# dylanpeifer/deepgroebner

Measured on NVIDIA B200. Metric: env_steps_per_sec, higher is better.
Workload: dtype u64 packed monomials + u32 GF(32003) coefficients (integer)

## Files before the change

### deepgroebner_b200/csrc/bb_device.cuh

```cuda
#pragma once
#include <cuda_runtime.h>
#include <stdint.h>

#include "../../include/bbenv.h"
#include "bb_layout.cuh"

#define BB_FULL 0xffffffffu
#ifndef BB_ADD_BASIS_INLINE
#define BB_ADD_BASIS_INLINE __noinline__
#endif
#define BB_GOLD 0x9E3779B97F4A7C15ULL
#define BB_GOLD2 0xD1B54A32D192ED03ULL

struct __align__(16) BBEnvState {
  int nG, nP, nT, status;
  int steps, adds, zero, nonzero;
  int rerolls, episode, truncated;
  unsigned sel_rng;
  unsigned long long trace_hash;
  unsigned long long rng;
  double disc_return, discount;
  unsigned long long pad2[2];
};

// ... 589 lines not shown
    if (two && i1 < m) { r1 = rlm[i1]; x1 = ridx[i1]; }
    pos = __popc(__ballot_sync(BB_FULL, i0 < m && r0 >= fk));
    if (two) pos += __popc(__ballot_sync(BB_FULL, i1 < m && r1 >= fk));
    __syncwarp();
    if (i0 < m && i0 >= pos) { rlm[i0 + 1] = r0; ridx[i0 + 1] = x0; }
    if (two && i1 < m && i1 >= pos) { rlm[i1 + 1] = r1; ridx[i1 + 1] = x1; }
    __syncwarp();
  } else if (H.sort_reducers) {
    int cnt = 0;
#pragma unroll 1
    for (int b0 = 0; b0 < m; b0 += 32) {
      const int r = b0 + lane;
      cnt += __popc(__ballot_sync(BB_FULL, r < m && rlm[r] >= fk));
    }
    pos = cnt;
#pragma unroll 1
    for (int hi = m; hi > pos; hi -= 32) {
      const int lo = hi - 32 > pos ? hi - 32 : pos;
      const int idx = lo + lane;
      const bool v = idx < hi;
      uint64_t k = 0; uint32_t ix = 0;
      if (v) { k = rlm[idx]; ix = ridx[idx]; }
      __syncwarp();
      if (v) { rlm[idx + 1] = k; ridx[idx + 1] = ix; }
      __syncwarp();
    }
  }
  if (lane == 0) {
    rlm[pos] = fk; ridx[pos] = (uint32_t)m;
    lm[m] = fk;
    GHeadMem* g = reinterpret_cast<GHeadMem*>(base + H.o_ghead) + m;
    if constexpr (TWO) {
      tk[0] = fk; tc[0] = c0;
      if (len > 1) { tk[1] = k1; tc[1] = c1; }
      else { k1 = 0ull; c1 = 0u; }
    }
    const uint32_t inv = bb_global(H.invtab)[TWO ? c0 : tc[0]];
    if constexpr (!TWO) {
      k1 = len > 1 ? tk[1] : 0ull;
      c1 = len > 1 ? tc[1] : 0u;
    }
    reinterpret_cast<uint4*>(g)[0] = make_uint4((uint32_t)fk, (uint32_t)(fk >> 32), (uint32_t)k1, (uint32_t)(k1 >> 32));
    reinterpret_cast<uint4*>(g)[1] = make_uint4(inv | (c1 << 16), (uint32_t)sug, (uint32_t)off, (uint32_t)len);
  }
  __syncwarp();
  return ((long long)emitted << 32) | (long long)nP;
}
template <int NV>
__device__ BB_ADD_BASIS_INLINE long long warp_add_basis(const BBParams& P, unsigned char* base, int m, int nP, int off, int len,
                                                        int sug) {
  return add_basis_body<NV, false>(P, base, m, nP, off, len, sug, 0ull, 0ull, 0u, 0u);
}
template <int NV>
__device__ BB_ADD_BASIS_INLINE long long warp_add_basis(const BBParams& P, unsigned char* base, int m, int nP, int off, int len,
                                                        int sug, uint64_t fk, uint64_t k1, uint32_t c0, uint32_t c1) {
  return add_basis_body<NV, true>(P, base, m, nP, off, len, sug, fk, k1, c0, c1);
}

__device__ __forceinline__ void warp_take_pair(const BBParams& P, Env& e, int row, uint32_t& pr, uint64_t& gam) {
  const int lane = bb_lane();
  uint32_t* pairs = ENV_PTR(uint32_t, e, P, o_pairs);
  uint64_t* plcm = ENV_PTR(uint64_t, e, P, o_plcm);
  pr = pairs[row];
  gam = plcm[row];
  __syncwarp();
#pragma unroll 1
  for (int b0 = row; b0 < e.nP - 1; b0 += 32) {
    const int idx = b0 + lane;
    const bool v = idx < e.nP - 1;
    uint32_t x = 0u; uint64_t y = 0ull;
    if (v) { x = pairs[idx + 1]; y = plcm[idx + 1]; }
    __syncwarp();
    if (v) { pairs[idx] = x; plcm[idx] = y; }
  }
  e.nP--;
}

template <int NV, bool TWO = false>
__device__ __forceinline__ int warp_step(const BBParams& P, Env& e, int row, uint32_t& pair, Ctr& ct) {
  typedef KL<NV> K;
  const BBField F = P.F;
  if ((unsigned)row >= (unsigned)e.nP) { e.status = BB_STATUS_BAD_ACTION; pair = 0xffffffffu; return 0; }
  uint32_t pr; uint64_t gam;
  warp_take_pair(P, e, row, pr, gam);
  const int i = pr & 0xffffu, j = pr >> 16;
  pair = pr;
  const GHeadMem* gh = ENV_PTR(GHeadMem, e, P, o_ghead);
  const GHead hf = load_head(gh + i), hg = load_head(gh + j);
  e.guard |= gam;
  ct.tread += hf.len + hg.len;
  Dividend h;
  h.k0 = h.k1 = 0; h.c0 = h.c1 = 0; h.n = 0; h.loc = -1;
  {
    const int cg0 = (int)(uint32_t)(gam >> K::dshift);
    const int sf = (int)hf.sug + (int)(uint32_t)(hf.lm >> K::dshift) - cg0, sg = (int)hg.sug + (int)(uint32_t)(hg.lm >> K::dshift) - cg0;
    h.sug = sf > sg ? sf : sg;
  }
  const uint64_t adjf = gam - hf.lm, adjg = gam - hg.lm;
  const uint32_t cg = F.p - hg.invlc;
  if (TWO || (hf.len <= 2 && hg.len <= 2)) {
    const uint64_t ka = hf.k1 + adjf, kb = hg.k1 + adjg;
    const bool hasA = hf.len == 2, hasB = hg.len == 2;
    if (hasA) e.guard |= ka;
    if (hasB) e.guard |= kb;
    tiny_merge(F, hasA, ka, bbf_mulmod(F, hf.c1, hf.invlc), hasB, kb, bbf_mulmod(F, hg.c1, cg), h);
  } else if constexpr (!TWO) {
    const uint64_t* tk = ENV_PTR(uint64_t, e, P, o_tkey);
// ... 506 lines not shown
```

### deepgroebner_b200/csrc/bb_kernels.cuh

```cuda
#pragma once
#include "bb_device.cuh"
#include "bb_policy.cuh"
#include "bb_streams.cuh"
#if defined(BBW_CLOCK) || defined(BBW_INSTR)
#include <cstdio>
#endif
#include "bb_wide.cuh"
#include "bb_rstreams.cuh"

#ifndef BB_WARPS
#define BB_WARPS 8
#endif
#define BB_THREADS (BB_WARPS * 32)
#ifndef BB_MIN_BLOCKS
#define BB_MIN_BLOCKS 3
#endif

#ifndef BB_ROLLOUT_MIN_BLOCKS
#define BB_ROLLOUT_MIN_BLOCKS 2
#endif

struct BBRunArgs {
  int strategy, episodes, seed_base;
  int sel_seed_base;
  int sel_seed_stride;
  int ep_base;
  int ep_offset;
  int nstaged;
  const int* seeds;
  int max_steps;
  double gamma;
  int compute_gb;
  bb_poly_sink gb_sink, basis_sink;
  bb_episode_stats* out;
  int32_t* trace;
  int trace_eps, trace_cap;
  int prepare_by_warp;
  int stream_kmax;
  int stream_regs;
  int ctl_reducers;
  int* queue;
  int* order;
  uint8_t* cost_key;
  int two_term;
};
#define BB_LPT_BUCKETS 256
#define BB_LPT_HIST 4

#define BB_PREP_S 16
struct BBPre {
  BBParams S;
  int depth;
  int* count;
  int* head;
  unsigned* rng;
  int* calls;
};

struct BBEpisodeAcc {
  unsigned long long th;
  double ret, disc;
  uint32_t sel_rng, pad;
};

struct BBValueArgs {
  int strategy;
  int rollouts;
  int sel_seed_base;
// ... 1 lines not shown
  double gamma;
  double* value;
  int* queue;
  int ntasks;
};

struct BBRolloutArgs {
  BBPolicy W;
  int T;
  unsigned long long counter0;
  int32_t* actions; float* logp; float* reward; uint8_t* done; int32_t* lengths;
  int32_t* obs; int pmax;
};

enum { BB_CMD_STEP = 1, BB_CMD_RESET = 2, BB_CMD_OBSERVE = 3, BB_CMD_STOP = 4 };
struct BBMailbox {
  volatile unsigned cmd_seq;
  unsigned cmd;
  int arg;
  int rows;
  unsigned pad0[12];
  volatile unsigned done_seq;
  volatile unsigned alive;
  int length;
  unsigned done;
  double reward;
  unsigned pad1[10];
};
static_assert(sizeof(BBMailbox) == 128, "mailbox header is two 64-byte lines");

struct BBKernelTable {
  int nvars, w, dw, dshift, eshift;
  cudaError_t (*reset)(const BBParams&, const uint8_t* mask, int nwarps, cudaStream_t);
  cudaError_t (*step)(const BBParams&, const int* actions, double* reward, uint8_t* done, const int* active, int nwarps,
                      cudaStream_t);
  cudaError_t (*step_obs)(const BBParams&, const int* actions, int action0, double* reward, uint8_t* done, int32_t* obs,
                          int32_t* lengths, int pmax, int pad, int do_step, const int* active, unsigned* ready, unsigned ticket,
                          int nwarps, cudaStream_t);
  cudaError_t (*serve)(const BBParams&, BBMailbox* mb, unsigned long long idle_ns, cudaStream_t);
  cudaError_t (*prefill)(const BBParams&, const BBParams& stage, int period, cudaStream_t);
  cudaError_t (*select)(const BBParams&, int strategy, int* actions, int nwarps, cudaStream_t);
  cudaError_t (*observe)(const BBParams&, int32_t* obs, int32_t* lengths, int pmax, int nwarps, cudaStream_t);
  cudaError_t (*final_gb)(const BBParams&, int slot, int* ok_out, cudaStream_t);
  cudaError_t (*prepare)(const BBParams& stage, const BBRunArgs&, cudaStream_t);
  cudaError_t (*run)(const BBParams&, const BBParams& stage, const BBRunArgs&, int nwarps, cudaStream_t);
  cudaError_t (*run_streams)(const BBParams&, const BBParams& stage, const BBRunArgs&, int nwarps, cudaStream_t);
  int (*streams_warps_per_sm)(void);
  cudaError_t (*run_wide)(const BBParams&, const BBParams& stage, const BBRunArgs&, int nctas, cudaStream_t);
  int (*wide_ctas_per_sm)(void);
  cudaError_t (*value)(const BBParams&, const BBParams& fork, const BBValueArgs&, int nwarps, cudaStream_t);
  cudaError_t (*policy)(const BBParams&, const BBPolicy&, unsigned long long counter, int32_t* actions, float* logp,
                        float* logits, int pmax, int nwarps, cudaStream_t);
  cudaError_t (*rollout)(const BBParams&, const BBRolloutArgs&, int nwarps, cudaStream_t);
  int (*run_blocks_per_sm)(void);
};

const BBKernelTable* bb_kernel_table(int nvars);

#ifdef BB_NV

__device__ __forceinline__ void counters_flush(const BBParams& P, unsigned long long (*sh)[CT_COUNT]) {
  __syncthreads();
  if (threadIdx.x < CT_COUNT) {
    unsigned long long s = 0;
#pragma unroll
    for (int w = 0; w < BB_WARPS; w++) s += sh[w][threadIdx.x];
    if (s) atomicAdd(&P.counters[threadIdx.x], s);
  }
}
__device__ __forceinline__ unsigned long long* counters_row(unsigned long long (*sh)[CT_COUNT]) {
  unsigned long long* row = sh[threadIdx.x >> 5];
  if (bb_lane() < CT_COUNT) row[bb_lane()] = 0ull;
  __syncwarp();
  return row;
}

template <int NV>
__device__ __noinline__ void warp_next_episode(const BBParams& P, int slot, unsigned long long* row);

template <int NV>
__global__ void __launch_bounds__(BB_THREADS, BB_MIN_BLOCKS) k_reset(const __grid_constant__ BBParams P, const uint8_t* mask) {
  __shared__ unsigned long long sh[BB_WARPS][CT_COUNT];
  hot_init(P);
  unsigned long long* row = counters_row(sh);
  const int slot = (blockIdx.x * BB_THREADS + threadIdx.x) >> 5;
  if (slot < P.num_envs && (!mask || mask[slot])) warp_next_episode<NV>(P, slot, row);
  counters_flush(P, sh);
}

template <int NV>
__device__ __forceinline__ double step_and_account(const BBParams& P, int slot, Env& e, int action, Ctr& ct,
                                                   unsigned long long* row) {
  uint32_t pr;
  const int g0 = e.nG;
  const int adds = warp_step<NV>(P, e, action, pr, ct);
  if (pr == 0xffffffffu) return 0.0;
  if (bb_lane() == 0) {
    const int pi = pr & 0xffffu, pj = pr >> 16;
    BBEnvState& S = P.st[slot];
    S.trace_hash = trace_hash_step(S.trace_hash, pr, adds);
    S.steps += 1; S.adds += adds;
    if (e.nG > g0) S.nonzero += 1; else S.zero += 1;
    row[CT_STEPS] += 1; row[CT_ADDS] += (unsigned)adds;
    row[e.nG > g0 ? CT_NONZERO : CT_ZERO] += 1;
    if (e.status == BB_STATUS_DONE) row[CT_EPISODES] += 1;
  }
  if (P.max_episode_length > 0 && e.status == BB_STATUS_RUNNING) {
// ... 533 lines not shown
      int steps = 0, adds = 0;
      if (lane == 0) { acc.th = 0ull; acc.ret = 0.0; acc.disc = 1.0; acc.sel_rng = rng_seed(A.sel_seed_base + (A.ep_offset + ep) * A.sel_seed_stride); }
      __syncwarp();
      run_episode<NV, STREAMS, TWO>(P, e, A.strategy, A.max_steps, A.gamma, acc, ct, steps, adds,
                               (A.trace && ep < A.trace_eps) ? reinterpret_cast<int4*>(A.trace) + (size_t)ep * A.trace_cap : nullptr,
                               A.trace_cap, &ws);
      const int nonzero = e.nG - g_start, zero = steps - nonzero;
      env_store(P, slot, e);
      __syncwarp();
      const GHeadMem* gh = ENV_PTR(GHeadMem, e, P, o_ghead);
      const unsigned long long bh = warp_terms_hash<NV>(ENV_PTR(uint64_t, e, P, o_tkey), ENV_PTR(uint32_t, e, P, o_tcoef),
                                                        e.nT, reinterpret_cast<const int*>(&gh[0].len),
                                                        (int)(sizeof(GHeadMem) / sizeof(int)), e.nG);
      unsigned long long gbh = 0; int gp = 0, gt = 0;
      int status = e.status;
      if (A.compute_gb && status == BB_STATUS_DONE) {
        if (warp_final_gb<NV>(P, slot, row)) {
          gp = P.gcount[2 * slot]; gt = P.gcount[2 * slot + 1];
          gbh = warp_terms_hash<NV>(P.gkey + (size_t)slot * P.max_terms, P.gcoef + (size_t)slot * P.max_terms, gt,
                                    P.glen + (size_t)slot * P.max_basis, 1, gp);
        } else {
          status = BB_STATUS_OVERFLOW_SCRATCH;
        }
      }
      if (EXPORT && (A.gb_sink.lens_dev || A.basis_sink.lens_dev)) warp_export_episode<NV>(P, A, slot, ep, status);
      if (lane == 0) {
        const unsigned long long th = acc.th; const double ret = acc.ret;
        bb_episode_stats o;
        o.steps = steps; o.additions = adds; o.zero_reductions = zero; o.nonzero_reductions = nonzero;
        o.nbasis = e.nG; o.nterms = e.nT; o.status = status; o.rerolls = S.st[b].rerolls;
        o.trace_hash = th; o.basis_hash = bh; o.gb_hash = gbh; o.gb_polys = gp; o.gb_terms = gt;
        o.discounted_return = ret;
        A.out[ep] = o;
        BBEnvState& St = P.st[slot];
        St.status = status; St.steps = steps; St.adds = adds; St.zero = zero; St.nonzero = nonzero; St.trace_hash = th;
        St.disc_return = ret; St.rerolls = o.rerolls;
        row[CT_STEPS] += (unsigned)steps; row[CT_ADDS] += (unsigned)adds; row[CT_NONZERO] += (unsigned)nonzero;
        row[CT_ZERO] += (unsigned)zero; row[CT_EPISODES] += 1;
      }
      ct.spill(row);
      __syncwarp();
    }
  }
  __syncthreads();
  if (threadIdx.x < CT_COUNT) {
    unsigned long long s = 0;
#pragma unroll
    for (int w = 0; w < WARPS; w++) s += sh[w][threadIdx.x];
    if (s) atomicAdd(&P.counters[threadIdx.x], s);
  }
}

template <int NV, bool EXPORT = false, bool TWO = false>
__global__ void __launch_bounds__(BB_THREADS, BB_MIN_BLOCKS) k_run(const __grid_constant__ BBParams P,
                                                                  const __grid_constant__ BBParams S,
                                                                  const __grid_constant__ BBRunArgs A) {
  run_worker<NV, false, BB_WARPS, EXPORT, TWO>(P, S, A);
}

#ifndef BBS_WARPS
#define BBS_WARPS 4
#endif
#ifndef BBS_MIN_CTAS
#define BBS_MIN_CTAS 2
#endif
template <int NV, bool EXPORT = false>
__global__ void __launch_bounds__(BBS_WARPS * 32, BBS_MIN_CTAS) k_run_streams(const __grid_constant__ BBParams P,
                                                                             const __grid_constant__ BBParams S,
                                                                             const __grid_constant__ BBRunArgs A) {
  run_worker<NV, true, BBS_WARPS, EXPORT>(P, S, A);
}

__device__ __forceinline__ void block_copy_words(uint32_t* __restrict__ d, const uint32_t* __restrict__ s, int n) {
  d = bb_global(d); s = bb_global(s);
#pragma unroll 1
  for (int t = threadIdx.x; t < n; t += BBW_THREADS) d[t] = s[t];
}

template <int NV>
__global__ void __launch_bounds__(BBW_THREADS, BBW_MIN_CTAS) k_run_wide(const __grid_constant__ BBParams P, const __grid_constant__ BBParams S,
                                                          const __grid_constant__ BBRunArgs A) {
  extern __shared__ __align__(16) unsigned char wide_smem[];
  __shared__ unsigned long long sh[1][CT_COUNT];
  __shared__ BBEpisodeAcc acc;
  __shared__ WideShared wsh;
  __shared__ int next_b;
  WideStreams& st = *reinterpret_cast<WideStreams*>(wide_smem);
  const int tid = threadIdx.x;
  const int slot = blockIdx.x;
  hot_init(P);
  if (tid < CT_COUNT) sh[0][tid] = 0ull;
  __syncthreads();
  unsigned long long* row = sh[0];
  Ctr ct; ct.clear();
  WideState ws;
  ws.clear(); ws.cz = 0;
#ifdef BBW_INSTR
  ws.n_rounds = ws.n_trounds = ws.sum_T = ws.n_consol = ws.n_crounds = ws.n_topen = 0;
#endif
#ifdef BBW_CLOCK
  ws.cw = ws.cb = ws.cp = ws.co = ws.s_sel = ws.s_take = ws.s_red = ws.s_upd = 0; ws.tl = clock64();
#endif
  ws.regs = A.stream_regs < BBW_SLOTS ? (A.stream_regs < 2 ? 2 : A.stream_regs) : BBW_SLOTS;
  ws.cbase = A.ctl_reducers >= 32 && A.ctl_reducers < 256 ? (A.ctl_reducers & ~31) : 256;
  ws.tcap = A.stream_kmax - ws.regs < 0 ? 0 : (A.stream_kmax - ws.regs < BBW_KMAX - BBW_THREADS ? A.stream_kmax - ws.regs : BBW_KMAX - BBW_THREADS);
  int half = 0;
  for (;;) {
    if (tid == 0) { int q = atomicAdd(A.queue, 1); next_b = q < A.episodes ? A.order[q] : -1; }
    __syncthreads();
    const int b = next_b;
// ... 198 lines not shown
      }
    }
    env_store(P, slot, e);
    ct.spill(row);
  }
  counters_flush(P, sh);
}

static inline int grid_for_warps(int nwarps) { return (nwarps + BB_WARPS - 1) / BB_WARPS; }

template <int NV>
struct BBLaunch {
  static cudaError_t reset(const BBParams& P, const uint8_t* mask, int nwarps, cudaStream_t s) {
    k_reset<NV><<<grid_for_warps(nwarps), BB_THREADS, 0, s>>>(P, mask);
    return cudaGetLastError();
  }
  static cudaError_t step(const BBParams& P, const int* actions, double* reward, uint8_t* done, const int* active, int nwarps,
                          cudaStream_t s) {
    k_step<NV><<<grid_for_warps(nwarps), BB_THREADS, 0, s>>>(P, actions, reward, done, active);
    return cudaGetLastError();
  }
  static cudaError_t step_obs(const BBParams& P, const int* actions, int action0, double* reward, uint8_t* done, int32_t* obs,
                              int32_t* lengths, int pmax, int pad, int do_step, const int* active, unsigned* ready,
                              unsigned ticket, int nwarps, cudaStream_t s) {
    k_step_obs<NV><<<grid_for_warps(nwarps), BB_THREADS, 0, s>>>(P, actions, action0, reward, done, obs, lengths, pmax, pad, do_step,
                                                                active, ready, ticket);
    return cudaGetLastError();
  }
  static cudaError_t serve(const BBParams& P, BBMailbox* mb, unsigned long long idle_ns, cudaStream_t s) {
    k_serve<NV><<<1, 32, 0, s>>>(P, mb, idle_ns);
    return cudaGetLastError();
  }
  static cudaError_t prefill(const BBParams& P, const BBParams& S, int period, cudaStream_t s) {
    k_prefill<NV><<<(P.num_envs + BB_PREP_THREADS - 1) / BB_PREP_THREADS, BB_PREP_THREADS, 0, s>>>(P, S, period);
    return cudaGetLastError();
  }
  static cudaError_t select(const BBParams& P, int strategy, int* actions, int nwarps, cudaStream_t s) {
    k_select<NV><<<grid_for_warps(nwarps), BB_THREADS, 0, s>>>(P, strategy, actions);
    return cudaGetLastError();
  }
  static cudaError_t observe(const BBParams& P, int32_t* obs, int32_t* lengths, int pmax, int nwarps, cudaStream_t s) {
    k_observe<NV><<<grid_for_warps(nwarps), BB_THREADS, 0, s>>>(P, obs, lengths, pmax);
    return cudaGetLastError();
  }
  static cudaError_t final_gb(const BBParams& P, int slot, int* ok_out, cudaStream_t s) {
    k_final_gb<NV><<<1, 32, 0, s>>>(P, slot, ok_out);
    return cudaGetLastError();
  }
  static void same_carveout() {
    static bool done = false;
    if (done) return;
    done = true;
    const int pct = 7;
    cudaFuncSetAttribute(k_run<NV>, cudaFuncAttributePreferredSharedMemoryCarveout, pct);
    cudaFuncSetAttribute(k_run<NV, true>, cudaFuncAttributePreferredSharedMemoryCarveout, pct);
    cudaFuncSetAttribute(k_run<NV, false, true>, cudaFuncAttributePreferredSharedMemoryCarveout, pct);
    cudaFuncSetAttribute(k_run<NV, true, true>, cudaFuncAttributePreferredSharedMemoryCarveout, pct);
    cudaFuncSetAttribute(k_prepare<NV>, cudaFuncAttributePreferredSharedMemoryCarveout, pct);
    cudaFuncSetAttribute(k_prepare_lanes<NV>, cudaFuncAttributePreferredSharedMemoryCarveout, pct);
    cudaFuncSetAttribute(k_order<NV>, cudaFuncAttributePreferredSharedMemoryCarveout, pct);
  }
  static cudaError_t prepare(const BBParams& S, const BBRunArgs& A, cudaStream_t s) {
    same_carveout();
    if (S.dist.enabled && S.dist.kind == 0 && S.dist.s <= BB_PREP_S && !A.prepare_by_warp)
      k_prepare_lanes<NV><<<(A.episodes + BB_PREP_THREADS - 1) / BB_PREP_THREADS, BB_PREP_THREADS, 0, s>>>(S, A);
    else
      k_prepare<NV><<<grid_for_warps(A.episodes), BB_THREADS, 0, s>>>(S, A);
    k_order<NV><<<std::min(64, (A.episodes + 1023) / 1024), BB_LPT_BUCKETS, 0, s>>>(A);
    return cudaGetLastError();
  }
  static cudaError_t run(const BBParams& P, const BBParams& S, const BBRunArgs& A, int nwarps, cudaStream_t s) {
    same_carveout();
    const bool ex = A.gb_sink.lens_dev || A.basis_sink.lens_dev;
    if (A.two_term) {
      if (ex) k_run<NV, true, true><<<grid_for_warps(nwarps), BB_THREADS, 0, s>>>(P, S, A);
      else k_run<NV, false, true><<<grid_for_warps(nwarps), BB_THREADS, 0, s>>>(P, S, A);
    } else {
      if (ex) k_run<NV, true><<<grid_for_warps(nwarps), BB_THREADS, 0, s>>>(P, S, A);
      else k_run<NV><<<grid_for_warps(nwarps), BB_THREADS, 0, s>>>(P, S, A);
    }
    return cudaGetLastError();
  }
  static size_t streams_smem() { return 0; }
  static int streams_warps_per_sm() {
    const size_t sm = streams_smem();
    if (cudaFuncSetAttribute(k_run_streams<NV>, cudaFuncAttributeMaxDynamicSharedMemorySize, (int)sm) != cudaSuccess) return 0;
    int blocks = 0;
    if (cudaOccupancyMaxActiveBlocksPerMultiprocessor(&blocks, k_run_streams<NV>, BBS_WARPS * 32, sm) != cudaSuccess) return 0;
    return blocks * BBS_WARPS;
  }
  static cudaError_t run_streams(const BBParams& P, const BBParams& S, const BBRunArgs& A, int nwarps, cudaStream_t s) {
    const size_t sm = streams_smem();
    const bool ex = A.gb_sink.lens_dev || A.basis_sink.lens_dev;
    cudaError_t e = cudaFuncSetAttribute(ex ? k_run_streams<NV, true> : k_run_streams<NV>,
                                         cudaFuncAttributeMaxDynamicSharedMemorySize, (int)sm);
    if (e != cudaSuccess) return e;
    if (ex) k_run_streams<NV, true><<<(nwarps + BBS_WARPS - 1) / BBS_WARPS, BBS_WARPS * 32, sm, s>>>(P, S, A);
    else k_run_streams<NV><<<(nwarps + BBS_WARPS - 1) / BBS_WARPS, BBS_WARPS * 32, sm, s>>>(P, S, A);
    return cudaGetLastError();
  }
  static int wide_ctas_per_sm() {
    const size_t sm = sizeof(WideStreams);
    if (cudaFuncSetAttribute(k_run_wide<NV>, cudaFuncAttributeMaxDynamicSharedMemorySize, (int)sm) != cudaSuccess) return 0;
    int blocks = 0;
    if (cudaOccupancyMaxActiveBlocksPerMultiprocessor(&blocks, k_run_wide<NV>, BBW_THREADS, sm) != cudaSuccess) return 0;
    return blocks;
  }
  static cudaError_t run_wide(const BBParams& P, const BBParams& S, const BBRunArgs& A, int nctas, cudaStream_t s) {
    const size_t sm = sizeof(WideStreams);
    cudaError_t e = cudaFuncSetAttribute(k_run_wide<NV>, cudaFuncAttributeMaxDynamicSharedMemorySize, (int)sm);
    if (e != cudaSuccess) return e;
    k_run_wide<NV><<<nctas, BBW_THREADS, sm, s>>>(P, S, A);
    return cudaGetLastError();
  }
  static cudaError_t value(const BBParams& P, const BBParams& F, const BBValueArgs& A, int nwarps, cudaStream_t s) {
    k_value<NV><<<grid_for_warps(nwarps), BB_THREADS, 0, s>>>(P, F, A);
    return cudaGetLastError();
  }
  static size_t policy_smem(const BBParams& P, int hidden) { return sizeof(float) * (size_t)policy_smem_floats(P.cols, hidden); }
  template <int UPL>
  static cudaError_t policy_upl(const BBParams& P, const BBPolicy& W, unsigned long long counter, int32_t* actions, float* logp,
                                float* logits, int pmax, int g, size_t sm, cudaStream_t s) {
    if (sm > 48 * 1024) {
      cudaError_t e = cudaFuncSetAttribute(k_policy<NV, UPL>, cudaFuncAttributeMaxDynamicSharedMemorySize, (int)sm);
      if (e != cudaSuccess) return e;
    }
    k_policy<NV, UPL><<<g, BB_THREADS, sm, s>>>(P, W, counter, actions, logp, logits, pmax);
    return cudaGetLastError();
  }
  static cudaError_t policy(const BBParams& P, const BBPolicy& W, unsigned long long counter, int32_t* actions, float* logp,
                            float* logits, int pmax, int nwarps, cudaStream_t s) {
    const size_t sm = policy_smem(P, W.hidden);
    const int g = grid_for_warps(nwarps);
    switch (W.hidden >> 5) {
      case 1: return policy_upl<1>(P, W, counter, actions, logp, logits, pmax, g, sm, s);
      case 2: return policy_upl<2>(P, W, counter, actions, logp, logits, pmax, g, sm, s);
      case 4: return policy_upl<4>(P, W, counter, actions, logp, logits, pmax, g, sm, s);
      case 8: return policy_upl<8>(P, W, counter, actions, logp, logits, pmax, g, sm, s);
    }
    return cudaErrorInvalidValue;
  }
  template <int UPL>
  static cudaError_t rollout_upl(const BBParams& P, const BBRolloutArgs& A, int g, size_t sm, cudaStream_t s) {
    if (sm > 48 * 1024) {
      cudaError_t e = cudaFuncSetAttribute(k_rollout<NV, UPL>, cudaFuncAttributeMaxDynamicSharedMemorySize, (int)sm);
      if (e != cudaSuccess) return e;
    }
    k_rollout<NV, UPL><<<g, BB_THREADS, sm, s>>>(P, A);
    return cudaGetLastError();
  }
  static cudaError_t rollout(const BBParams& P, const BBRolloutArgs& A, int nwarps, cudaStream_t s) {
    const size_t sm = policy_smem(P, A.W.hidden);
    const int g = grid_for_warps(nwarps);
    switch (A.W.hidden >> 5) {
      case 1: return rollout_upl<1>(P, A, g, sm, s);
      case 2: return rollout_upl<2>(P, A, g, sm, s);
      case 4: return rollout_upl<4>(P, A, g, sm, s);
      case 8: return rollout_upl<8>(P, A, g, sm, s);
    }
    return cudaErrorInvalidValue;
  }
  static int run_blocks_per_sm() {
    int blocks = 0;
    if (cudaOccupancyMaxActiveBlocksPerMultiprocessor(&blocks, k_run<NV>, BB_THREADS, 0) != cudaSuccess) return -1;
    return blocks;
  }
  static const BBKernelTable* table() {
    static const BBKernelTable t = {NV, KL<NV>::w, KL<NV>::dw, KL<NV>::dshift, KL<NV>::eshift,
                                    &reset, &step, &step_obs, &serve, &prefill, &select, &observe, &final_gb, &prepare, &run, &run_streams, &streams_warps_per_sm, &run_wide, &wide_ctas_per_sm, &value, &policy,
                                    &rollout,
                                    &run_blocks_per_sm};
    return &t;
  }
};
#endif
```

### deepgroebner_b200/csrc/bbenv.cu

```cuda
#include <cuda_runtime.h>
#include <emmintrin.h>

#include <algorithm>
#include <cmath>
#include <cstdio>
#include <cstring>
#include <string>
#include <vector>

#include "bb_kernels.cuh"

__global__ void __launch_bounds__(BB_THREADS) k_seed(BBParams P, const int* seeds, int base, int selection) {
  int e = blockIdx.x * blockDim.x + threadIdx.x;
  if (e >= P.num_envs) return;
  const uint32_t x = rng_seed(seeds ? seeds[e] : base + e);
  if (selection) P.st[e].sel_rng = x;
  else {
    P.st[e].rng = x;
    if (P.pre) { P.pre->count[e] = 0; P.pre->head[e] = 0; P.pre->rng[e] = x; }
  }
}

__global__ void __launch_bounds__(BB_THREADS) k_pre_flush(BBParams P, int only_env) {
  int e = blockIdx.x * blockDim.x + threadIdx.x;
// ... 121 lines not shown
  BBLayout L;
  const BBKernelTable* K;
  int sm_count;
  std::vector<void*> allocs;
  std::string err;
  int* d_queue;
  int* d_ok;
  struct Stage {
    int cap;
    std::vector<void*> allocs;
    unsigned char* arena; BBEnvState* st;
    uint64_t* in_key; uint32_t* in_coef; int* in_off; int* in_np;
    int* order; uint8_t* cost_key;
    int* queue;
    cudaEvent_t prepared;
    cudaEvent_t consumed;
    int episodes, seed_base; const int32_t* seeds;
    unsigned long long serial;
  } stage[BB_STAGE_SETS];
  unsigned long long stage_serial;
  int stage_next;
  cudaStream_t side;
  cudaEvent_t ev_entry;
  int timing; cudaEvent_t ev_t[3];
  int fork_cap;
  std::vector<void*> fork_allocs;
  unsigned char* fork_arena; BBEnvState* fork_st;
  unsigned char* host_stage; unsigned char* dev_stage; size_t stage_bytes;
  int sel_seed_stride;
  int episode_offset;
  int nstaged;
  int* d_seeds; int* h_seeds; cudaEvent_t ev_seeds;
  struct Bank {
    bool ready;
    unsigned char* arena; BBEnvState* st;
    uint64_t* gkey; uint32_t* gcoef; int* glen; int* gcount; uint64_t* grlm; uint32_t* gridx; uint32_t* gflag;
    cudaEvent_t done;
    cudaStream_t stream;
    unsigned long long serial;
  } bank[BB_BANKS];
  int* d_active;
  int compaction;
  unsigned ticket;
  int pre_depth;
  bool pre_ready;
  BBPre* d_pre; BBParams preS; std::vector<void*> pre_allocs;
  int serve_on;
  bool serving;
  BBMailbox* mb; size_t mb_bytes;
  unsigned serve_seq;
  cudaStream_t serve_stream; cudaEvent_t ev_serve;
  int prepare_by_warp;
  int two_term;
  int wide_mode;
  std::vector<double> cp;
  std::vector<char> staged;
};

static thread_local std::string g_create_err;

static int fail(bb_handle* h, const std::string& msg, int code = -1) {
  if (h) h->err = msg; else g_create_err = msg;
  return code;
}
#define CK(call)                                                                                      \
  do {                                                                                                \
    cudaError_t _e = (call);                                                                          \
    if (_e != cudaSuccess)                                                                            \
      return fail(h, std::string(#call) + ": " + cudaGetErrorString(_e), -2);                         \
  } while (0)

template <class T>
static cudaError_t dev_alloc(bb_handle* h, T** p, size_t count) {
  void* q = nullptr;
  cudaError_t e = cudaMalloc(&q, count * sizeof(T) + 16);
  if (e != cudaSuccess) return e;
  h->allocs.push_back(q);
  *p = (T*)q;
  return cudaMemset(q, 0, count * sizeof(T) + 16);
}

static bool layout_arena(BBParams& P) {
  size_t o = 0;
  auto take = [&o](size_t bytes) { size_t at = o; o = (o + bytes + 31) & ~(size_t)31; return (unsigned)at; };
  P.o_ghead = take(sizeof(GHeadMem) * (size_t)P.max_basis);
  P.o_lm = take(8 * (size_t)P.max_basis);
  P.o_rlm = take(8 * (size_t)P.max_basis);
  P.o_lscr = take(8 * (size_t)P.max_basis);
  P.o_plcm = take(8 * (size_t)P.max_pairs);
  P.o_tkey = take(8 * (size_t)P.max_terms);
  P.o_hkey = take(8 * 2 * (size_t)P.max_poly_terms);
  P.o_ridx = take(4 * (size_t)P.max_basis);
  P.o_pairs = take(4 * (size_t)P.max_pairs);
  P.o_tcoef = take(4 * (size_t)P.max_terms);
  P.o_hcoef = take(4 * 2 * (size_t)P.max_poly_terms);
  P.o_logit = take(4 * (size_t)P.max_pairs);
  if (o >= ((size_t)1 << 31)) return false;
  P.slot_stride = (o + 127) & ~(size_t)127;
  return true;
}

static inline int grid_for_warps_host(int nwarps) { return (nwarps + BB_WARPS - 1) / BB_WARPS; }

#define BB_SERVE_IDLE_NS 10000000ull

static inline void serve_post(bb_handle* h, unsigned cmd, int arg, int pmax, int pad) {
// ... 100 lines not shown
    if (e == cudaSuccess) { h->pre_allocs.push_back(*out); e = cudaMemset(*out, 0, bytes + 16); }
    return e;
  };
  BBPre Q;
  CK(alloc((void**)&S.arena, n * S.slot_stride));
  CK(alloc((void**)&S.st, n * sizeof(BBEnvState)));
  S.num_envs = (int)n;
  S.in_key = nullptr; S.in_coef = nullptr; S.in_off = nullptr; S.in_np = nullptr;
  CK(alloc((void**)&Q.count, N * sizeof(int)));
  CK(alloc((void**)&Q.head, N * sizeof(int)));
  CK(alloc((void**)&Q.rng, N * sizeof(unsigned)));
  CK(alloc((void**)&Q.calls, sizeof(int)));
  CK(alloc((void**)&h->d_pre, sizeof(BBPre)));
  Q.S = S; Q.depth = h->pre_depth;
  CK(cudaMemcpy(h->d_pre, &Q, sizeof Q, cudaMemcpyHostToDevice));
  CK(cudaDeviceSynchronize());
  h->preS = S;
  h->P.pre = h->d_pre;
  h->pre_ready = true;
  k_pre_flush<<<(P.num_envs + BB_THREADS - 1) / BB_THREADS, BB_THREADS, 0, s>>>(h->P, -1);
  CK(cudaGetLastError());
  return 0;
}

static int pre_refill(bb_handle* h, cudaStream_t s, bool now) {
  int rc = pre_setup(h, s);
  if (rc < 0 || !h->pre_ready) return rc;
  CK(h->K->prefill(h->P, h->preS, now ? 0 : 4 * h->pre_depth, s));
  return 0;
}

#define ENTER(h)                                                                                      \
  do {                                                                                                \
    CK(cudaSetDevice((h)->cfg.device));                                                               \
    if ((h)->serving) { int _rc = serve_stop(h); if (_rc < 0) return _rc; }                           \
  } while (0)

extern "C" {

int bb_abi_version(void) { return BB_ABI_VERSION; }

const char* bb_last_error(const bb_handle* h) { return h ? h->err.c_str() : g_create_err.c_str(); }
int bb_cols(const bb_handle* h) { return h->P.cols; }
int bb_num_envs(const bb_handle* h) { return h->P.num_envs; }
int bb_sm_count(const bb_handle* h) { return h->sm_count; }
uint64_t bb_hash_item(uint64_t x, uint64_t pos) { return bb_hash_item_impl(x, pos); }

int bb_resident_envs(int device, int nvars) {
  int sms = 0;
  const BBKernelTable* K = bb_kernel_table(nvars);
  if (!K) return -1;
  if (cudaDeviceGetAttribute(&sms, cudaDevAttrMultiProcessorCount, device) != cudaSuccess) return -1;
  if (cudaSetDevice(device) != cudaSuccess) return -1;
  const int blocks = K->run_blocks_per_sm();
  if (blocks <= 0) return -1;
  return sms * blocks * BB_WARPS;
}

void bb_destroy(bb_handle* h) {
  if (!h) return;
  cudaSetDevice(h->cfg.device);
  serve_stop(h);
  if (h->mb) cudaFreeHost(h->mb);
  if (h->serve_stream) cudaStreamDestroy(h->serve_stream);
  if (h->ev_serve) cudaEventDestroy(h->ev_serve);
  for (void* p : h->allocs) cudaFree(p);
  for (int b = 0; b < BB_STAGE_SETS; b++) {
    for (void* p : h->stage[b].allocs) cudaFree(p);
    if (h->stage[b].prepared) cudaEventDestroy(h->stage[b].prepared);
    if (h->stage[b].consumed) cudaEventDestroy(h->stage[b].consumed);
  }
  for (int b = 0; b < BB_BANKS; b++) if (h->bank[b].done) cudaEventDestroy(h->bank[b].done);
  if (h->side) cudaStreamDestroy(h->side);
  if (h->ev_entry) cudaEventDestroy(h->ev_entry);
  if (h->ev_seeds) cudaEventDestroy(h->ev_seeds);
  for (int t = 0; t < 3; t++) if (h->ev_t[t]) cudaEventDestroy(h->ev_t[t]);
  if (h->h_seeds) cudaFreeHost(h->h_seeds);
  for (void* p : h->fork_allocs) cudaFree(p);
  for (void* p : h->pre_allocs) cudaFree(p);
  if (h->host_stage) cudaFreeHost(h->host_stage);
  if (h->dev_stage) cudaFree(h->dev_stage);
  delete h;
}

int bb_create(const bb_config* cfg, bb_handle** out) {
  bb_handle* h = nullptr;
  if (!cfg || !out) return fail(h, "bb_create: null argument");
  if (cfg->abi_version != BB_ABI_VERSION) return fail(h, "bb_create: ABI version mismatch");
  if (cfg->nvars < 1 || cfg->nvars > 8) return fail(h, "bb_create: nvars must be in 1..8");
  if (cfg->prime < 3 || cfg->prime > 65535) return fail(h, "bb_create: prime must be in 3..65535");
  for (int q = 2; q * q <= cfg->prime; q++)
    if (cfg->prime % q == 0) return fail(h, "bb_create: prime is not prime");
  if (cfg->k < 1) return fail(h, "bb_create: k must be >= 1");
  if (cfg->num_envs < 1) return fail(h, "bb_create: num_envs must be >= 1");
  if (cfg->max_basis < 2 || cfg->max_basis > 65535) return fail(h, "bb_create: max_basis must be in 2..65535");
  if (cfg->max_pairs < 1 || cfg->max_pairs > 65536) return fail(h, "bb_create: max_pairs must be in 1..65536");
  if (cfg->max_terms < 2 || cfg->max_poly_terms < 1 || cfg->max_gens < 1 || cfg->max_gen_terms < 1)
    return fail(h, "bb_create: capacities must be positive");
  if (cfg->max_gens > cfg->max_basis) return fail(h, "bb_create: max_gens exceeds max_basis");
  if ((unsigned)cfg->elimination > 2u || (unsigned)cfg->rewards > 1u) return fail(h, "bb_create: bad enum value");
  int ndev = 0;
  if (cudaGetDeviceCount(&ndev) != cudaSuccess || ndev == 0)
    return fail(h, "bb_create: no CUDA device available (this library has no CPU fallback)", -3);
  if (cfg->device < 0 || cfg->device >= ndev) return fail(h, "bb_create: bad device ordinal");
  h = new bb_handle();
  h->cfg = *cfg;
  h->d_queue = nullptr; h->d_ok = nullptr;
  for (int b = 0; b < BB_STAGE_SETS; b++) {
    bb_handle::Stage& T = h->stage[b];
    T.cap = 0; T.arena = nullptr; T.st = nullptr; T.in_key = nullptr; T.in_coef = nullptr; T.in_off = nullptr; T.in_np = nullptr;
    T.order = nullptr; T.cost_key = nullptr; T.queue = nullptr; T.prepared = nullptr; T.consumed = nullptr;
    T.episodes = 0; T.seed_base = 0; T.seeds = nullptr; T.serial = 0;
  }
  for (int b = 0; b < BB_BANKS; b++) { h->bank[b].ready = false; h->bank[b].done = nullptr; h->bank[b].stream = nullptr; h->bank[b].serial = 0; }
  h->stage_next = 0; h->stage_serial = 0; h->side = nullptr; h->ev_entry = nullptr; h->timing = 0;
  h->ev_t[0] = h->ev_t[1] = h->ev_t[2] = nullptr;
  h->episode_offset = 0; h->nstaged = 0; h->d_seeds = nullptr; h->h_seeds = nullptr; h->ev_seeds = nullptr;
  h->d_active = nullptr; h->compaction = 1; h->ticket = 0u;
  h->pre_depth = cfg->num_envs >= BB_PRE_MIN_ENVS ? BB_PRE_DEPTH : 0; h->pre_ready = false; h->d_pre = nullptr;
  h->serve_on = cfg->num_envs == 1 ? 1 : 0; h->serving = false; h->mb = nullptr; h->mb_bytes = 0; h->serve_seq = 0u;
  h->serve_stream = nullptr; h->ev_serve = nullptr;
  h->fork_cap = 0; h->fork_arena = nullptr; h->fork_st = nullptr;
  h->wide_mode = -1;
  h->prepare_by_warp = 0;
  h->two_term = 1;
  h->host_stage = nullptr; h->dev_stage = nullptr; h->stage_bytes = 0;
  h->sel_seed_stride = 1;
  auto bail = [&](int code) { g_create_err = h->err; bb_destroy(h); return code; };
#define CKC(call)                                                                                     \
  do {                                                                                                \
    cudaError_t _e = (call);                                                                          \
    if (_e != cudaSuccess) { h->err = std::string(#call) + ": " + cudaGetErrorString(_e); return bail(-2); } \
  } while (0)
  CKC(cudaSetDevice(cfg->device));
  cudaDeviceProp prop;
  CKC(cudaGetDeviceProperties(&prop, cfg->device));
  h->sm_count = prop.multiProcessorCount;
  BBParams& P = h->P;
  memset(&P, 0, sizeof P);
  h->L = bb_make_layout(cfg->nvars, (uint32_t)cfg->prime);
  h->K = bb_kernel_table(cfg->nvars);
  if (!h->K || h->K->w != h->L.w || h->K->dw != h->L.dw || h->K->dshift != h->L.dshift || h->K->eshift != h->L.eshift) {
    h->err = "bb_create: kernel table / layout mismatch"; return bail(-6);
  }
  P.F.p = h->L.p; P.F.mu = h->L.mu; P.nvars = cfg->nvars;
  P.num_envs = cfg->num_envs; P.k = cfg->k; P.cols = 2 * cfg->nvars * cfg->k;
  P.elimination = cfg->elimination; P.rewards = cfg->rewards;
  P.sort_input = cfg->sort_input ? 1 : 0; P.sort_reducers = cfg->sort_reducers ? 1 : 0;
  P.max_basis = cfg->max_basis; P.max_pairs = cfg->max_pairs; P.max_terms = (cfg->max_terms + 7) & ~7;
  P.max_poly_terms = cfg->max_poly_terms; P.max_gens = cfg->max_gens; P.max_gen_terms = cfg->max_gen_terms;
  P.obs_nv = cfg->nvars; P.max_episode_length = 0;
  const size_t N = (size_t)cfg->num_envs;
  if (!layout_arena(P)) { h->err = "bb_create: per-environment arena exceeds 2 GiB"; return bail(-1); }
  CKC(dev_alloc(h, &P.arena, N * P.slot_stride));
  CKC(dev_alloc(h, &P.st, N));
  CKC(dev_alloc(h, &P.in_key, N * P.max_gen_terms));
  CKC(dev_alloc(h, &P.in_coef, N * P.max_gen_terms));
  CKC(dev_alloc(h, &P.in_off, N * (P.max_gens + 1)));
  CKC(dev_alloc(h, &P.in_np, N));
  CKC(dev_alloc(h, &P.gkey, N * P.max_terms));
  CKC(dev_alloc(h, &P.gcoef, N * P.max_terms));
  CKC(dev_alloc(h, &P.glen, N * P.max_basis));
  CKC(dev_alloc(h, &P.gcount, N * 2));
  CKC(dev_alloc(h, &P.grlm, N * P.max_basis));
  CKC(dev_alloc(h, &P.gridx, N * P.max_basis));
  CKC(dev_alloc(h, &P.gflag, N * P.max_basis));
  CKC(dev_alloc(h, &P.counters, (size_t)CT_COUNT));
  {
    uint16_t* tab = nullptr;
    CKC(dev_alloc(h, &tab, (size_t)cfg->prime));
    k_invtab<<<(cfg->prime + BB_THREADS - 1) / BB_THREADS, BB_THREADS>>>(P.F, tab);
    CKC(cudaGetLastError());
    P.invtab = tab;
  }
  CKC(dev_alloc(h, &h->d_queue, (size_t)4));
  CKC(dev_alloc(h, &h->d_ok, (size_t)4));
  CKC(dev_alloc(h, &h->d_seeds, N));
  CKC(dev_alloc(h, &h->d_active, std::max(N + 1, (size_t)16)));
  for (int b = 0; b < BB_BANKS; b++) CKC(cudaEventCreateWithFlags(&h->bank[b].done, cudaEventDisableTiming));
  h->bank[0].ready = true;
  h->bank[0].arena = P.arena; h->bank[0].st = P.st; h->bank[0].gkey = P.gkey; h->bank[0].gcoef = P.gcoef; h->bank[0].glen = P.glen;
  h->bank[0].gcount = P.gcount; h->bank[0].grlm = P.grlm; h->bank[0].gridx = P.gridx; h->bank[0].gflag = P.gflag;
  CKC(cudaHostAlloc((void**)&h->h_seeds, sizeof(int) * N, cudaHostAllocDefault));
  CKC(cudaEventCreateWithFlags(&h->ev_seeds, cudaEventDisableTiming));
  CKC(cudaEventCreateWithFlags(&h->ev_entry, cudaEventDisableTiming));
  CKC(cudaStreamCreateWithFlags(&h->side, cudaStreamNonBlocking));
  CKC(cudaStreamCreateWithFlags(&h->serve_stream, cudaStreamNonBlocking));
  CKC(cudaEventCreateWithFlags(&h->ev_serve, cudaEventDisableTiming));
  for (int b = 0; b < BB_STAGE_SETS; b++) {
    CKC(dev_alloc(h, &h->stage[b].queue, (size_t)(BB_LPT_HIST + 2 * BB_LPT_BUCKETS)));
    CKC(cudaEventCreateWithFlags(&h->stage[b].prepared, cudaEventDisableTiming));
    CKC(cudaEventCreateWithFlags(&h->stage[b].consumed, cudaEventDisableTiming));
  }
  for (int t = 0; t < 3; t++) CKC(cudaEventCreate(&h->ev_t[t]));
  k_seed<<<(cfg->num_envs + BB_THREADS - 1) / BB_THREADS, BB_THREADS>>>(P, nullptr, 0, 0);
  k_seed<<<(cfg->num_envs + BB_THREADS - 1) / BB_THREADS, BB_THREADS>>>(P, nullptr, 0, 1);
// ... 500 lines not shown
    PB.grlm = B.grlm; PB.gridx = B.gridx; PB.gflag = B.gflag;
  }
  int which = -1;
  {
    const int count0 = std::min(BB_RUN_BATCH, episodes);
    for (int b = 0; b < BB_STAGE_SETS; b++) {
      const bb_handle::Stage& T = h->stage[b];
      const bool m = T.episodes == count0 && nbatch == 1 && T.seed_base == seed_base && T.seeds == seeds_dev;
      if (m && (which < 0 || T.serial < h->stage[which].serial)) which = b;
    }
    const bool ready = which >= 0;
    if (!ready) which = stage_take(h);
    bb_handle::Stage& T = h->stage[which];
    if (h->timing) CK(cudaEventRecord(h->ev_t[0], s));
    if (ready) CK(cudaStreamWaitEvent(s, T.prepared, 0));
    else {
      rc = enqueue_prepare(h, which, 0, count0, seed_base, seeds_dev, s);
      if (rc < 0) return rc;
    }
    T.episodes = 0;
    if (h->timing) CK(cudaEventRecord(h->ev_t[1], s));
  }
  if (nbatch > 1) CK(cudaEventRecord(h->ev_entry, s));
  for (const bb_poly_sink* k : {gb, basis})
    if (k) CK(cudaMemsetAsync(k->where_dev, 0xff, sizeof(int64_t) * 2 * (size_t)episodes, s));
  for (int bi = 0; bi < nbatch; bi++) {
    const int base = bi * BB_RUN_BATCH, count = std::min(BB_RUN_BATCH, episodes - base);
    int next = -1;
    if (bi + 1 < nbatch) {
      const int nbase = base + BB_RUN_BATCH;
      if (bi == 0) CK(cudaStreamWaitEvent(h->side, h->ev_entry, 0));
      next = stage_take(h);
      rc = enqueue_prepare(h, next, nbase, std::min(BB_RUN_BATCH, episodes - nbase), seed_base, seeds_dev, h->side);
      if (rc < 0) return rc;
    }
    BBParams S;
    rc = stage_params(h, which, h->stage[which].cap, S);
    if (rc < 0) return rc;
    BBRunArgs A;
    prepare_args(h, which, base, count, seed_base, seeds_dev, A);
    A.strategy = strategy; A.sel_seed_base = sel_seed_base; A.sel_seed_stride = h->sel_seed_stride;
    A.max_steps = max_steps; A.gamma = gamma; A.compute_gb = compute_gb; A.out = stats_dev;
    if (gb) A.gb_sink = *gb;
    if (basis) A.basis_sink = *basis;
    A.trace = trace_dev; A.trace_eps = trace_dev ? trace_episodes : 0; A.trace_cap = trace_cap;
    A.stream_kmax = (h->wide_mode == 2 || h->wide_mode == 5) ? 6 : ((h->wide_mode == 3 || h->wide_mode == 6) ? 48 : BBS_KMAX);
    A.stream_regs = h->wide_mode == 7 ? 8 : A.stream_kmax;
    A.ctl_reducers = h->wide_mode == 8 ? 32 : 256;
    A.two_term = h->two_term && h->P.dist.enabled && h->P.dist.kind == 0;
    if (bi > 0) CK(cudaStreamWaitEvent(s, h->stage[which].prepared, 0));
    const int workers = std::min(h->P.num_envs, count);
    if (streams && h->wide_mode >= 4 && h->wide_mode <= 6) CK(h->K->run_streams(PB, S, A, workers, s));
    else if (streams) CK(h->K->run_wide(PB, S, A, std::min(workers, wide_ctas), s));
    else CK(h->K->run(PB, S, A, workers, s));
    CK(cudaEventRecord(h->stage[which].consumed, s));
    CK(cudaEventRecord(h->bank[bk].done, s));
    if (h->timing && bi == 0) CK(cudaEventRecord(h->ev_t[2], s));
    which = next;
  }
  return 0;
}

int bb_set_timing(bb_handle* h, int on) {
  if (!h) return -1;
  h->timing = on ? 1 : 0;
  return 0;
}

int bb_last_run_ms(bb_handle* h, float* prepare_ms, float* run_ms) {
  if (!h) return -1;
  if (!h->timing) return fail(h, "bb_last_run_ms: timing is off (bb_set_timing)");
  ENTER(h);
  CK(cudaEventSynchronize(h->ev_t[2]));
  float a = 0.f, b = 0.f;
  CK(cudaEventElapsedTime(&a, h->ev_t[0], h->ev_t[1]));
  CK(cudaEventElapsedTime(&b, h->ev_t[1], h->ev_t[2]));
  if (prepare_ms) *prepare_ms = a;
  if (run_ms) *run_ms = b;
  return 0;
}

int bb_set_episode_offset(bb_handle* h, int offset) {
  if (!h) return -1;
  if (offset < 0) return fail(h, "bb_set_episode_offset: negative offset");
  h->episode_offset = offset;
  return 0;
}

static int fork_params(bb_handle* h, int workers, BBParams& F) {
  const BBParams& P = h->P;
  F = P;
  if (workers > h->fork_cap) {
    for (void* p : h->fork_allocs) cudaFree(p);
    h->fork_allocs.clear();
    h->fork_cap = 0;
    auto alloc = [&](void** out, size_t bytes) {
      cudaError_t e = cudaMalloc(out, bytes + 16);
      if (e == cudaSuccess) { h->fork_allocs.push_back(*out); e = cudaMemset(*out, 0, bytes + 16); }
      return e;
    };
    CK(alloc((void**)&h->fork_arena, (size_t)workers * P.slot_stride));
    CK(alloc((void**)&h->fork_st, (size_t)workers * sizeof(BBEnvState)));
    h->fork_cap = workers;
  }
  F.arena = h->fork_arena; F.st = h->fork_st; F.num_envs = workers;
  return 0;
}

int bb_value(bb_handle* h, int strategy, double gamma, int rollouts, int sel_seed_base, int max_steps,
             double* value_dev, void* stream) {
  if (!h) return -1;
  if (!value_dev) return fail(h, "bb_value: null output");
  if (strategy == BB_VALUE_SAMPLE) rollouts = rollouts > 0 ? rollouts : 101;
  else if ((unsigned)strategy > 8u) return fail(h, "bb_value: bad strategy");
  else if (strategy != BB_SELECT_RANDOM || rollouts < 1) rollouts = 1;
  ENTER(h);
  cudaStream_t s = (cudaStream_t)stream;
  const int N = h->P.num_envs;
  const long long ntasks = (long long)N * rollouts;
  if (ntasks > 0x7fffffffLL) return fail(h, "bb_value: too many rollouts");
  int workers = h->K->run_blocks_per_sm() * h->sm_count * BB_WARPS;
  const long long by_mem = (long long)(((size_t)8 << 30) / h->P.slot_stride);
  workers = (int)std::max(1LL, std::min((long long)workers, std::min(ntasks, by_mem)));
  BBParams F;
  if (workers > h->fork_cap) CK(cudaStreamSynchronize(s));
  int rc = fork_params(h, std::max(workers, h->fork_cap), F);
  if (rc < 0) return rc;
  F.num_envs = workers;
  BBValueArgs A;
  A.strategy = strategy; A.rollouts = rollouts; A.sel_seed_base = sel_seed_base; A.max_steps = max_steps;
  A.gamma = gamma; A.value = value_dev; A.queue = h->d_queue; A.ntasks = (int)ntasks;
  CK(cudaMemsetAsync(h->d_queue, 0, sizeof(int), s));
  k_fill_double<<<(N + BB_THREADS - 1) / BB_THREADS, BB_THREADS, 0, s>>>(value_dev, N, -__builtin_inf());
  CK(cudaGetLastError());
  CK(h->K->value(h->P, F, A, workers, s));
  return 0;
}

int bb_copy_env(bb_handle* dst, int dst_env, bb_handle* src, int src_env, void* stream) {
  bb_handle* h = dst;
  if (!dst || !src) return -1;
  if (dst_env < 0 || dst_env >= dst->P.num_envs || src_env < 0 || src_env >= src->P.num_envs)
    return fail(h, "bb_copy_env: environment index out of range");
  const bb_config &a = dst->cfg, &b = src->cfg;
  if (a.device != b.device || a.nvars != b.nvars || a.prime != b.prime || a.max_basis != b.max_basis ||
      a.max_pairs != b.max_pairs || a.max_terms != b.max_terms || a.max_poly_terms != b.max_poly_terms ||
      a.max_gens != b.max_gens || a.max_gen_terms != b.max_gen_terms)
    return fail(h, "bb_copy_env: handles differ in device, field, variables or capacities");
  if (dst == src && dst_env == src_env) return 0;
  CK(cudaSetDevice(a.device));
  if (dst->serving) { int rc = serve_stop(dst); if (rc < 0) return rc; }
  if (src->serving && serve_stop(src) < 0) return fail(h, "bb_copy_env: " + src->err);
  cudaStream_t s = (cudaStream_t)stream;
  const BBParams &D = dst->P, &S = src->P;
  CK(cudaMemcpyAsync(D.arena + (size_t)dst_env * D.slot_stride, S.arena + (size_t)src_env * S.slot_stride, S.slot_stride,
                     cudaMemcpyDeviceToDevice, s));
  CK(cudaMemcpyAsync(D.st + dst_env, S.st + src_env, sizeof(BBEnvState), cudaMemcpyDeviceToDevice, s));
  CK(cudaMemcpyAsync(D.in_key + (size_t)dst_env * D.max_gen_terms, S.in_key + (size_t)src_env * S.max_gen_terms,
                     sizeof(uint64_t) * S.max_gen_terms, cudaMemcpyDeviceToDevice, s));
  CK(cudaMemcpyAsync(D.in_coef + (size_t)dst_env * D.max_gen_terms, S.in_coef + (size_t)src_env * S.max_gen_terms,
                     sizeof(uint32_t) * S.max_gen_terms, cudaMemcpyDeviceToDevice, s));
  CK(cudaMemcpyAsync(D.in_off + (size_t)dst_env * (D.max_gens + 1), S.in_off + (size_t)src_env * (S.max_gens + 1),
                     sizeof(int) * (S.max_gens + 1), cudaMemcpyDeviceToDevice, s));
  CK(cudaMemcpyAsync(D.in_np + dst_env, S.in_np + src_env, sizeof(int), cudaMemcpyDeviceToDevice, s));
  if (dst->pre_ready) {
    k_pre_flush<<<(D.num_envs + BB_THREADS - 1) / BB_THREADS, BB_THREADS, 0, s>>>(D, dst_env);
    CK(cudaGetLastError());
  }
  return 0;
}

int bb_discount(bb_handle* h, int N, int T, const double* x_dev, const uint8_t* done_dev, double gam, double* out_dev,
                void* stream) {
  if (!h) return -1;
// ... 219 lines not shown
```

Before: 1.079 billion.

## Give two-term runner its own launch bounds and cap launch to one resident wave

Adds separate launch bounds for the two-term k_run variant (min 4 CTAs per SM instead of 3) and force-inlines the two-term warp_add_basis. It also computes per-variant resident warp capacity from the occupancy API and caps the number of run workers to a single resident wave. The aim is higher occupancy for the two-term path and no tail waves of workers. The tighter register budget may cause spills, and force-inlining may grow code size and register pressure.

```diff
diff --git a/deepgroebner_b200/csrc/bb_device.cuh b/deepgroebner_b200/csrc/bb_device.cuh
--- a/deepgroebner_b200/csrc/bb_device.cuh
+++ b/deepgroebner_b200/csrc/bb_device.cuh
@@ -665,7 +665,7 @@
   return add_basis_body<NV, false>(P, base, m, nP, off, len, sug, 0ull, 0ull, 0u, 0u);
 }
 template <int NV>
-__device__ BB_ADD_BASIS_INLINE long long warp_add_basis(const BBParams& P, unsigned char* base, int m, int nP, int off, int len,
+__device__ __forceinline__ long long warp_add_basis(const BBParams& P, unsigned char* base, int m, int nP, int off, int len,
                                                         int sug, uint64_t fk, uint64_t k1, uint32_t c0, uint32_t c1) {
   return add_basis_body<NV, true>(P, base, m, nP, off, len, sug, fk, k1, c0, c1);
 }
diff --git a/deepgroebner_b200/csrc/bb_kernels.cuh b/deepgroebner_b200/csrc/bb_kernels.cuh
--- a/deepgroebner_b200/csrc/bb_kernels.cuh
+++ b/deepgroebner_b200/csrc/bb_kernels.cuh
@@ -14,6 +14,12 @@
 #define BB_THREADS (BB_WARPS * 32)
 #ifndef BB_MIN_BLOCKS
 #define BB_MIN_BLOCKS 3
+#endif
+#ifndef BB_TWO_WARPS
+#define BB_TWO_WARPS BB_WARPS
+#endif
+#ifndef BB_TWO_MIN_BLOCKS
+#define BB_TWO_MIN_BLOCKS 4
 #endif
 
 #ifndef BB_ROLLOUT_MIN_BLOCKS
@@ -121,7 +127,7 @@
   cudaError_t (*policy)(const BBParams&, const BBPolicy&, unsigned long long counter, int32_t* actions, float* logp,
                         float* logits, int pmax, int nwarps, cudaStream_t);
   cudaError_t (*rollout)(const BBParams&, const BBRolloutArgs&, int nwarps, cudaStream_t);
-  int (*run_blocks_per_sm)(void);
+  int (*run_warps_per_sm)(int two);
 };
 
 const BBKernelTable* bb_kernel_table(int nvars);
@@ -761,10 +767,9 @@
 }
 
 template <int NV, bool EXPORT = false, bool TWO = false>
-__global__ void __launch_bounds__(BB_THREADS, BB_MIN_BLOCKS) k_run(const __grid_constant__ BBParams P,
-                                                                  const __grid_constant__ BBParams S,
-                                                                  const __grid_constant__ BBRunArgs A) {
-  run_worker<NV, false, BB_WARPS, EXPORT, TWO>(P, S, A);
+__global__ void __launch_bounds__(TWO ? BB_TWO_WARPS * 32 : BB_THREADS, TWO ? BB_TWO_MIN_BLOCKS : BB_MIN_BLOCKS)
+k_run(const __grid_constant__ BBParams P, const __grid_constant__ BBParams S, const __grid_constant__ BBRunArgs A) {
+  run_worker<NV, false, TWO ? BB_TWO_WARPS : BB_WARPS, EXPORT, TWO>(P, S, A);
 }
 
 #ifndef BBS_WARPS
@@ -1069,6 +1074,8 @@
     if (done) return;
     done = true;
     const int pct = 7;
+    static_assert(BB_TWO_MIN_BLOCKS * (BB_TWO_WARPS * (CT_COUNT * 8 + sizeof(BBEpisodeAcc)) + 1024) <= 16 * 1024,
+                  "the 16 KB split holds BB_TWO_MIN_BLOCKS two-term runner CTAs");
     cudaFuncSetAttribute(k_run<NV>, cudaFuncAttributePreferredSharedMemoryCarveout, pct);
     cudaFuncSetAttribute(k_run<NV, true>, cudaFuncAttributePreferredSharedMemoryCarveout, pct);
     cudaFuncSetAttribute(k_run<NV, false, true>, cudaFuncAttributePreferredSharedMemoryCarveout, pct);
@@ -1090,8 +1097,9 @@
     same_carveout();
     const bool ex = A.gb_sink.lens_dev || A.basis_sink.lens_dev;
     if (A.two_term) {
-      if (ex) k_run<NV, true, true><<<grid_for_warps(nwarps), BB_THREADS, 0, s>>>(P, S, A);
-      else k_run<NV, false, true><<<grid_for_warps(nwarps), BB_THREADS, 0, s>>>(P, S, A);
+      const int g = (nwarps + BB_TWO_WARPS - 1) / BB_TWO_WARPS;
+      if (ex) k_run<NV, true, true><<<g, BB_TWO_WARPS * 32, 0, s>>>(P, S, A);
+      else k_run<NV, false, true><<<g, BB_TWO_WARPS * 32, 0, s>>>(P, S, A);
     } else {
       if (ex) k_run<NV, true><<<grid_for_warps(nwarps), BB_THREADS, 0, s>>>(P, S, A);
       else k_run<NV><<<grid_for_warps(nwarps), BB_THREADS, 0, s>>>(P, S, A);
@@ -1177,16 +1185,19 @@
     }
     return cudaErrorInvalidValue;
   }
-  static int run_blocks_per_sm() {
+  static int run_warps_per_sm(int two) {
+    same_carveout();
     int blocks = 0;
-    if (cudaOccupancyMaxActiveBlocksPerMultiprocessor(&blocks, k_run<NV>, BB_THREADS, 0) != cudaSuccess) return -1;
-    return blocks;
+    const cudaError_t e = two ? cudaOccupancyMaxActiveBlocksPerMultiprocessor(&blocks, k_run<NV, false, true>, BB_TWO_WARPS * 32, 0)
+                              : cudaOccupancyMaxActiveBlocksPerMultiprocessor(&blocks, k_run<NV>, BB_THREADS, 0);
+    if (e != cudaSuccess) return -1;
+    return blocks * (two ? BB_TWO_WARPS : BB_WARPS);
   }
   static const BBKernelTable* table() {
     static const BBKernelTable t = {NV, KL<NV>::w, KL<NV>::dw, KL<NV>::dshift, KL<NV>::eshift,
                                     &reset, &step, &step_obs, &serve, &prefill, &select, &observe, &final_gb, &prepare, &run, &run_streams, &streams_warps_per_sm, &run_wide, &wide_ctas_per_sm, &value, &policy,
                                     &rollout,
-                                    &run_blocks_per_sm};
+                                    &run_warps_per_sm};
     return &t;
   }
 };
diff --git a/deepgroebner_b200/csrc/bbenv.cu b/deepgroebner_b200/csrc/bbenv.cu
--- a/deepgroebner_b200/csrc/bbenv.cu
+++ b/deepgroebner_b200/csrc/bbenv.cu
@@ -197,6 +197,7 @@
   cudaStream_t serve_stream; cudaEvent_t ev_serve;
   int prepare_by_warp;
   int two_term;
+  int run_wave[2];
   int wide_mode;
   std::vector<double> cp;
   std::vector<char> staged;
@@ -403,9 +404,9 @@
   if (!K) return -1;
   if (cudaDeviceGetAttribute(&sms, cudaDevAttrMultiProcessorCount, device) != cudaSuccess) return -1;
   if (cudaSetDevice(device) != cudaSuccess) return -1;
-  const int blocks = K->run_blocks_per_sm();
-  if (blocks <= 0) return -1;
-  return sms * blocks * BB_WARPS;
+  const int w0 = K->run_warps_per_sm(0), w1 = K->run_warps_per_sm(1);
+  if (w0 <= 0 || w1 <= 0) return -1;
+  return sms * std::max(w0, w1);
 }
 
 void bb_destroy(bb_handle* h) {
@@ -493,6 +494,11 @@
   h->K = bb_kernel_table(cfg->nvars);
   if (!h->K || h->K->w != h->L.w || h->K->dw != h->L.dw || h->K->dshift != h->L.dshift || h->K->eshift != h->L.eshift) {
     h->err = "bb_create: kernel table / layout mismatch"; return bail(-6);
+  }
+  for (int two = 0; two < 2; two++) {
+    const int w = h->K->run_warps_per_sm(two);
+    if (w <= 0) { h->err = "bb_create: k_run does not fit on the device"; return bail(-2); }
+    h->run_wave[two] = w * h->sm_count;
   }
   P.F.p = h->L.p; P.F.mu = h->L.mu; P.nvars = cfg->nvars;
   P.num_envs = cfg->num_envs; P.k = cfg->k; P.cols = 2 * cfg->nvars * cfg->k;
@@ -1099,7 +1105,7 @@
     const int workers = std::min(h->P.num_envs, count);
     if (streams && h->wide_mode >= 4 && h->wide_mode <= 6) CK(h->K->run_streams(PB, S, A, workers, s));
     else if (streams) CK(h->K->run_wide(PB, S, A, std::min(workers, wide_ctas), s));
-    else CK(h->K->run(PB, S, A, workers, s));
+    else CK(h->K->run(PB, S, A, std::min(workers, h->run_wave[A.two_term]), s));
     CK(cudaEventRecord(h->stage[which].consumed, s));
     CK(cudaEventRecord(h->bank[bk].done, s));
     if (h->timing && bi == 0) CK(cudaEventRecord(h->ev_t[2], s));
@@ -1166,7 +1172,7 @@
   const int N = h->P.num_envs;
   const long long ntasks = (long long)N * rollouts;
   if (ntasks > 0x7fffffffLL) return fail(h, "bb_value: too many rollouts");
-  int workers = h->K->run_blocks_per_sm() * h->sm_count * BB_WARPS;
+  int workers = h->run_wave[0];
   const long long by_mem = (long long)(((size_t)8 << 30) / h->P.slot_stride);
   workers = (int)std::max(1LL, std::min((long long)workers, std::min(ntasks, by_mem)));
   BBParams F;
```

Result: faster. 1.153 billion (median of 6 runs) (+6.9%).
